# zeynelacikgoez/PyAudioLocalization

Hardware: AMD Instinct MI355X
Metric: mic-pair GCC-PHAT correlations/s @44.1kHz·1s (higher is better)
Workload: dtype f64; 1 GPU; metric run: 64 frame(s)/step/GPU x 64 mics x 44100 samples @ 44100 Hz, 2016 pairs/frame, max_expected_delay=0.05; n=88199 = 89 x 991: prime-factor inverse, Rader row DFTs (cyclic convolutions of 990 points in LDS) + dense column DFTs; mics=64, samples=44100, pairs_per_frame=2016, fused_column_statistics=default, finishing_column_pass=default, rader_columns=default, gather=none, split=frames, parallelism=frames sharded over 1 GPU(s)

## Files before the change

### pyaudiolocalization_amd/csrc/engine.h

```cpp
#pragma once
#include <hip/hip_runtime.h>

#include <cstdarg>
#include <cstdint>
#include <cstdio>
#include <map>
#include <string>
#include <tuple>
#include <vector>

#include "../../include/pal_hip.h"
#include "fin_scratch.h"
#include "fft_core.h"
#include "pair_route.h"
#include "plan_geometry.h"
#include "peak_types.h"
#include "resample_math.h"

namespace pal {

struct FinArgs;

struct Conv {
  ConvGeom g;
// ... 23 lines not shown
  int n = 0;
  int H = 0;
  int lin = 0;
  int nout = 0;
  cd* w = nullptr;
  Conv fwd;
  Conv inv;
  Pfa pfa;
  long long used = 0;
  size_t spec_stride() const { return pfa.on() ? size_t(pfa.rows()) * size_t(pfa.n2) : size_t(H); }
};

struct ProfileSlot {
  double ms = 0;
  int64_t launches = 0;
};

enum Ws : int {
  kWsWork = 0,
  kWsCorr = 1,
  kWsSpectra = 2,
  kWsQuads = 3,
  kWsStageIn = 4, kWsStageTable = 5, kWsStageOut = 6, kWsStagePairs = 15,
  kWsStatus = 7,
  kWsPeaks0 = 8, kWsPeaks1 = 9, kWsPeaks2 = 12,
  kWsBootRows = 10, kWsBootRound = 11, kWsBootPeaks = 13,
  kWsZeroRows = 14,
  kWsFin0 = 16, kWsFin1 = 17, kWsFin2 = 18,
  kWsFlags = 19, kWsFlagQuads = 20, kWsFlagTable = 21,
  kWsSolve = 22,
  kWsBlockTable = 23,
  kWsResample = 24,
  kWsClosure = 25,
  kWsCount = 26
};
constexpr Ws peak_scratch_slot(int slot) { return slot == 0 ? kWsPeaks0 : (slot == 1 ? kWsPeaks1 : kWsPeaks2); }
constexpr Ws fin_scratch_slot(int slot) { return Ws(kWsFin0 + slot); }

struct Engine {
  int device = 0;
  int cu_count = 256;
  hipStream_t stream = nullptr;
  hipStream_t stream2 = nullptr;
  hipStream_t stream3 = nullptr;
  hipStream_t stream_of(int slot) const { return slot == 0 ? stream : (slot == 1 ? stream2 : stream3); }
  hipEvent_t ev_fork = nullptr, ev_join2 = nullptr, ev_join3 = nullptr;
  hipEvent_t ev_fin = nullptr;
  int fin_serialize(hipStream_t on);
  int fin_done(hipStream_t on);
  bool fin_pending = false;
  bool fin_serial = false;
  bool rows_lean = true;
  long long rows_lean_min = 200000;
  bool lean_store = true;
  int debug_memo = 0;
  bool one_stream = false;
  PlanSwitches plan_sw;
  bool xcd_rows = true;
  bool rows_shared = true;
  std::string err;
  static constexpr int kDefaultChunk = 128;
  int chunk = kDefaultChunk;
  bool chunk_auto = true;
  int pair_group(int n) const {
    if (!chunk_auto) return chunk;
    const long long g = (1ll << 30) / (16ll * (n > 0 ? n : 1));
    return int(g < 32 ? 32 : (g > 240 ? 240 : g));
  }
  std::map<std::tuple<int, int, int>, Plan> plans;
  struct XConv { Conv conv; long long used = 0; };
// ... 70 lines not shown
  int solve_positions_impl(const pal_pair_record* d_tables, int B, int M, const int32_t* lengths, const double* mics, const double* calib,
                           const double* weights, const double* extra_starts, const pal_solve_params* prm, pal_position_record* out,
                           int loss, double f_scale, double* pair_weights);
  int tdoa_closure_dev(const pal_pair_record* d_tables, int B, int M, const int32_t* lengths, int32_t tol, int32_t min_votes, int32_t weight_mode,
                       int32_t* d_votes, int32_t* d_mic_closed, double* d_weights, pal_closure_frame* d_summary);
  int closure_check(int B, int M, const int32_t* lengths, int32_t tol, int32_t min_votes, int32_t weight_mode);
  int32_t* solve_idx = nullptr;
  int solve_idx_M = 0;
  std::vector<double> rs_win;
  std::vector<ResampleTap> rs_host;
  int rs_num_table = 0;
  double rs_ratio = 0;
  int peaks(const double* corr, size_t stride, int rows, int n, int n2, const pal_phat_params& prm,
            pal_pair_record* table, int32_t* ksel_multi, int slot);
  int peaks_setup(const double* corr, size_t stride, int rows, int n, int n2, const pal_phat_params& prm, int blocks, int grid_n2, int slot, PeakArgs& a);
  int peaks_finish(PeakArgs& a, int rows, pal_pair_record* table, int32_t* ksel_multi, int slot);
  int pfa_rows(const Plan& pl, const cd* permuted, const int4* quads, int G, cd* Y, hipStream_t on);
  int fin_setup(const Plan& pl, int rows, int nblk, int grid_rows, const pal_phat_params& prm, int n2, pal_pair_record* table,
                int* need, int slot, PeakArgs& a, struct FinArgs& fa, unsigned& nwg, int G);
  int rows_lean_group(const Plan& pl, const double* corr, size_t stride, int G, int rows, const pal_phat_params& prm, int n2,
                      pal_pair_record* table, int* need, int slot);
  int pfa_pair_group_fin(const Plan& pl, const cd* permuted, const int4* quads, int G, int rows, cd* Y, const int* zero_rows,
                         const pal_phat_params& prm, int n2, pal_pair_record* table, int* need, int slot,
                         double* corr = nullptr, size_t stride = 0);
  int pfa_pair_group_fused(const Plan& pl, const cd* permuted, const int4* quads, int G, int rows, cd* Y, double* corr, size_t stride,
                           const int* zero_rows, const pal_phat_params& prm, int n2, pal_pair_record* table, int32_t* ksel_multi, int slot);
  bool pfa_forward_applies(const Plan& pl, int len) const;
  int pfa_forward_spectra(Plan& pl, const double* frames, size_t frame_stride, int rows, int len, cd* spectra, const int* flags);
  bool pfa_forward = true;
  bool fin_cols = true;
  unsigned fin_epoch[3] = {};
  FinKey fin_key[3];
  unsigned fin_wrap = kFinEpochWrap;
  int fin_giveup = 0;
  bool fuse_peaks = true;
};

struct ProfScope {
  Engine* e;
  int slot;
  hipEvent_t a = nullptr;
  hipStream_t on;
  ProfScope(Engine* eng, const char* name, hipStream_t s = nullptr) : e(eng), slot(-1), on(s ? s : eng->stream) {
    if (e->profiling && e->prof_gate) {
      slot = e->prof_slot(name);
      e->prof_begin(slot, &a, on);
    }
  }
  ~ProfScope() {
    if (slot >= 0) e->prof_end(slot, a, on);
  }
};

#define PAL_TRY(expr)                \
  do {                               \
    int _rc = (expr);                \
    if (_rc != PAL_OK) return _rc;   \
  } while (0)

#define PAL_HIP(expr) PAL_TRY(check((expr), #expr))

}
```

### pyaudiolocalization_amd/csrc/pair_route.h

```cpp
#pragma once

namespace pal {

constexpr int kColsOwn = 62;

struct RouteIn {
  int n, nout; bool split; int n1, n2, nch, lm; bool r89;
  bool table, corr, multi; long long npairs;
  bool stored_only;
  int num_peaks, threshold_method; double threshold_multiplier;
  bool fin_cols, fuse_peaks, lean_store, rows_lean; long long rows_lean_min;
};

enum class RouteTransform { kFinish, kLeanStore, kFused, kPfa, kFourStep };
enum class RouteStats { kNone, kPass, kRowsLean, kThreeLaunches };

struct PairRoute {
  RouteTransform transform;
  RouteStats stats;
  bool flags_pairs() const { return transform == RouteTransform::kFinish || transform == RouteTransform::kLeanStore || stats == RouteStats::kRowsLean; }
};

inline int fin_blocks(int n2, int nch) { return (n2 + (nch <= 1 ? 4 : 1) * kColsOwn - 1) / ((nch <= 1 ? 4 : 1) * kColsOwn); }

inline bool nohist(int threshold_method, double threshold_multiplier) {
  return threshold_method > 0 || (threshold_multiplier >= 0 && threshold_multiplier <= 2.0);
}

inline PairRoute pair_route(const RouteIn& f) {
  const bool lean_peak = f.fin_cols && !f.stored_only && f.num_peaks == 1 && !f.multi;
  const bool no_hist = nohist(f.threshold_method, f.threshold_multiplier);
  const int nblk = fin_blocks(f.n2, f.nch);
  if (f.table && f.fuse_peaks && f.split && f.nch >= 1 && f.nch <= 4 && f.n2 >= 3) {
    bool cols_ok = f.r89 || (f.nch >= 2 && f.nch <= 4) || (f.nch <= 1 && f.lm <= 13);
    if (!f.r89 && nblk < 12) cols_ok = false;
    if (lean_peak && !f.corr && f.n2 >= 256 && cols_ok) return {RouteTransform::kFinish, RouteStats::kPass};
    if (f.lean_store && lean_peak && nblk >= 12 && no_hist) return {RouteTransform::kLeanStore, RouteStats::kPass};
    return {RouteTransform::kFused, RouteStats::kPass};
  }
  const RouteTransform tr = f.split ? RouteTransform::kPfa : RouteTransform::kFourStep;
  if (!f.table) return {tr, RouteStats::kNone};
  const bool lean = f.rows_lean && lean_peak && f.npairs >= f.rows_lean_min && no_hist && f.nout == f.n && f.n >= 4096 && f.n <= 50000;
  return {tr, lean ? RouteStats::kRowsLean : RouteStats::kThreeLaunches};
}

}
```

### pyaudiolocalization_amd/csrc/pal_api.hip

```cpp
#include <dlfcn.h>

#include <cmath>
#include <cstring>

#include "engine.h"

namespace pal {

static std::string g_create_error;

int Engine::fail(int code, const char* fmt, ...) {
  char buf[512];
  va_list ap;
  va_start(ap, fmt);
  vsnprintf(buf, sizeof buf, fmt, ap);
  va_end(ap);
  err = buf;
  return code;
}

int Engine::check(hipError_t e, const char* what) {
  if (e == hipSuccess) return PAL_OK;
  const int code = e == hipErrorOutOfMemory ? PAL_ERR_NOMEM : PAL_ERR_HIP;
  return fail(code, "%s: %s", what, hipGetErrorString(e));
// ... 264 lines not shown
  if (env) e->plan_sw.allow_pfa = atoi(env) != 0;
  env = getenv("PAL_RADER");
  if (env) e->plan_sw.allow_rader = atoi(env) != 0;
  env = getenv("PAL_PFA_BIG");
  if (env) e->plan_sw.allow_big = atoi(env) != 0;
  env = getenv("PAL_FOUR_REG");
  if (env) e->plan_sw.four_reg = atoi(env) != 0;
  env = getenv("PAL_XCD_ROWS");
  if (env) e->xcd_rows = atoi(env) != 0;
  env = getenv("PAL_ROWS_SHARED");
  if (env) e->rows_shared = atoi(env) != 0;
  env = getenv("PAL_PFA_FWD");
  if (env) e->pfa_forward = atoi(env) != 0;
  env = getenv("PAL_FUSED");
  if (env) e->fuse_peaks = atoi(env) != 0;
  env = getenv("PAL_R89");
  if (env) e->plan_sw.allow_r89 = atoi(env) != 0;
  env = getenv("PAL_FIN_SERIAL");
  if (env) e->fin_serial = atoi(env) != 0;
  env = getenv("PAL_FIN");
  if (env) e->fin_cols = atoi(env) != 0;
  env = getenv("PAL_ROWS_LEAN");
  if (env) e->rows_lean = atoi(env) != 0;
  env = getenv("PAL_PAIR_BLOCK");
  if (env) e->pair_block = atoi(env);
  env = getenv("PAL_ROWS_LEAN_MIN");
  if (env && atoll(env) >= 1) e->rows_lean_min = atoll(env);
  env = getenv("PAL_LEAN_STORE");
  if (env) e->lean_store = atoi(env) != 0;
  env = getenv("PAL_DEBUG_MEMO");
  if (env) e->debug_memo = atoi(env);
  env = getenv("PAL_DEBUG_FIN_WRAP");
  if (env && atoi(env) >= 2) e->fin_wrap = unsigned(atoi(env));
  env = getenv("PAL_DEBUG_FIN_GIVEUP");
  if (env) e->fin_giveup = atoi(env) != 0 ? 1 : 0;
  env = getenv("PAL_MAX_PLANS");
  if (env && atoi(env) >= 2) e->max_plans = atoi(env);
  *out = reinterpret_cast<pal_handle>(e);
  return PAL_OK;
}

void pal_destroy(pal_handle h) {
  if (!h) return;
  Engine* e = reinterpret_cast<Engine*>(h);
  hipSetDevice(e->device);
  pal_comm_destroy(h);
  (void)e->clear_plans();
  for (cd* p : e->stage_tw) if (p) hipFree(p);
  for (cd* p : e->stage_twc) if (p) hipFree(p);
  for (void* p : e->ws) if (p) hipFree(p);
  if (e->quads) hipFree(e->quads);
  if (e->quads_blk) hipFree(e->quads_blk);
  if (e->perm_blk) hipFree(e->perm_blk);
  if (e->solve_idx) hipFree(e->solve_idx);
  for (hipEvent_t ev : e->ev_pool) hipEventDestroy(ev);
  hipStreamDestroy(e->stream2);
  hipStreamDestroy(e->stream3);
  hipEventDestroy(e->ev_fork);
  hipEventDestroy(e->ev_join2);
  hipEventDestroy(e->ev_join3);
  hipEventDestroy(e->ev_fin);
  hipStreamDestroy(e->stream);
  delete e;
}

const char* pal_last_error(pal_handle h) {
// ... 468 lines not shown
```

### pyaudiolocalization_amd/csrc/pfa.hip

```cpp
#include <cmath>
#include <cstdlib>
#include <vector>

#include "pfa_kernels.h"
#include "pfa_rader.h"
#include "pfa_cols_stats.h"
#include "pfa_cols_fin.h"
#include "pfa_forward.h"
#include "pfa_big.h"

namespace pal {

#ifndef PAL_BIG13_PTS
#define PAL_BIG13_PTS 32
#endif
#ifndef PAL_BIG14_PTS
#define PAL_BIG14_PTS 32
#endif
constexpr int kBig13 = PAL_BIG13_PTS, kBig14 = PAL_BIG14_PTS;

static_assert(kColChunk == kPfaTC && kColUnroll == kPfaUnr && kRader89 == kR89, "plan_geometry.h against the column pass's constants");
static_assert(sizeof(RowStep) == sizeof(int2) && sizeof(Cplx) == sizeof(cd), "plan_geometry.h tables are uploaded as they are");

void Engine::free_pfa(Pfa& f) {
// ... 182 lines not shown
  return PAL_OK;
}

int Engine::fin_setup(const Plan& pl, int rows, int nblk, int grid_rows, const pal_phat_params& prm, int n2, pal_pair_record* table,
                      int* need, int slot, PeakArgs& a, FinArgs& fa, unsigned& nwg, int G) {
  const int n = pl.n;
  PAL_TRY(peaks_setup(nullptr, 0, rows, n, n2, prm, nblk, 0, slot, a));
  const FinLayout lay = fin_layout(pair_group(n), nblk, grid_rows);
  char* base = nullptr;
  PAL_TRY(scratch(fin_scratch_slot(slot), lay.total, &base));
  PAL_TRY(status_words(&fa.status));
  fa.table = table;
  fa.need = need;
  fa.done = reinterpret_cast<unsigned*>(base);
  FinKey key;
  key.gmax = pair_group(n);
  key.nblk = nblk;
  key.grid_rows = grid_rows;
  key.block = ws_bytes[fin_scratch_slot(slot)];
  if (fin_must_zero(fin_key[slot], key, fin_epoch[slot], fin_wrap)) {
    PAL_HIP(hipMemsetAsync(base, 0, key.block, stream_of(slot)));
    fin_key[slot] = key;
    fin_epoch[slot] = 0;
  }
  fa.epoch = ++fin_epoch[slot];
  fa.emax = reinterpret_cast<double*>(base + lay.off_emax);
  fa.parts = reinterpret_cast<FinPartial*>(base + lay.off_parts);
  fa.edge = reinterpret_cast<double*>(base + lay.off_edge);
  fa.giveup = fin_giveup;
  fa.pw = 1;
  fa.corr = nullptr;
  fa.stride = 0;
  fa.store_rows = 0;
  fa.windowed = std::isnan(prm.max_expected_delay) ? 0 : 1;
  fa.win_lo = 1;
  fa.win_hi = n - 2;
  if (fa.windowed) {
    const double med = prm.max_expected_delay, fs = prm.fs;
    long long k = -1;
    if (med >= 0) {
      const double est = med * fs;
      k = est < double(n) ? (long long)est + 2 : (long long)n;
      while (k >= 0 && !(std::fabs(double(k) / fs) <= med)) --k;
    }
    if (k < 0) { fa.win_lo = 1; fa.win_hi = 0; }
    else {
      const long long lo = (long long)(n2 - 1) - k, hi = (long long)(n2 - 1) + k;
      fa.win_lo = int(lo < 1 ? 1 : lo);
      fa.win_hi = int(hi > n - 2 ? n - 2 : hi);
    }
  }
  fa.cheb = a.method == 0 && nohist(prm.threshold_method, prm.threshold_multiplier) ? 1 : 0;
  nwg = 8u * unsigned((G + 7) / 8) * unsigned(nblk);
  return PAL_OK;
}

int Engine::rows_lean_group(const Plan& pl, const double* corr, size_t stride, int G, int rows, const pal_phat_params& prm, int n2,
                            pal_pair_record* table, int* need, int slot) {
  constexpr int NS = 22;
  const hipStream_t on = stream_of(slot);
  const int chunks = (pl.n + kColsOwn - 1) / kColsOwn;
  const int nblk = (chunks + 4 * NS - 1) / (4 * NS);
  PeakArgs a;
  FinArgs fa;
  unsigned nwg = 0;
  PAL_TRY(fin_setup(pl, rows, nblk, 1, prm, n2, table, need, slot, a, fa, nwg, G));
  fa.pw = 4;
  fa.corr = const_cast<double*>(corr);
  fa.stride = stride;
  ProfScope ps(this, "k_rows_lean", on);
  k_rows_lean<NS><<<dim3(nwg), dim3(256), 0, on>>>(corr, stride, G, nblk, a, fa, rows);
  PAL_HIP(hipGetLastError());
  return PAL_OK;
}

int Engine::pfa_pair_group_fin(const Plan& pl, const cd* permuted, const int4* quads, int G, int rows, cd* Y, const int* zero_rows,
                               const pal_phat_params& prm, int n2, pal_pair_record* table, int* need, int slot,
                               double* corr, size_t stride) {
  const Pfa& f = pl.pfa;
  const hipStream_t on = stream_of(slot);
  const bool shortcols = f.nch <= 1;
  const int nblk = fin_blocks(f.n2, f.nch);
  PeakArgs a;
  FinArgs fa;
  unsigned nwg = 0;
  PAL_TRY(fin_setup(pl, rows, nblk, f.n1, prm, n2, table, need, slot, a, fa, nwg, G));
  fa.corr = corr;
  fa.stride = stride;
  fa.store_rows = corr ? 1 : 0;
  PAL_TRY(pfa_rows(pl, permuted, quads, G, Y, on));
  {
    ProfScope ps(this, corr ? "k_pfa_cols_lean" : "k_pfa_cols_fin", on);
    const dim3 grid(nwg);
    const bool full = (f.n1 - 1) / 2 == f.nch * kPfaTC;
    const bool hist = !(a.method > 0 || fa.cheb);
    const int nw = f.nch == 2 ? 2 : (f.nch == 3 && !hist ? 3 : 4);
    FinSrc src{Y, f.T, static_cast<const Rader89Tab*>(f.r89_tab)};
    PAL_TRY(fin_serialize(on));
#define PAL_COLS_FIN(MODE, HI, FU, NW) k_pfa_cols_fin<MODE, kPfaTC, kPfaUnr, HI, FU, NW><<<grid, dim3(64 * NW), 0, on>>>(src, f.n1, f.n2, G, f.nch, nblk, zero_rows, a, fa, rows)
#define PAL_COLS_FIN_FU(MODE, HI, NW) do { if (full) PAL_COLS_FIN(MODE, HI, true, NW); else PAL_COLS_FIN(MODE, HI, false, NW); } while (0)
    if (!hist) fa.pw = shortcols ? 4 : nw;
    if (shortcols) { if (hist) PAL_COLS_FIN(kColsStrips, true, false, 4); else PAL_COLS_FIN(kColsStrips, false, false, 4); }
    else if (f.r89 && full && nw == 4) { if (hist) PAL_COLS_FIN(kColsRader89, true, true, 4); else PAL_COLS_FIN(kColsRader89, false, true, 4); }
    else if (nw == 3) PAL_COLS_FIN_FU(kColsDense, false, 3);
    else if (nw == 2) { if (hist) PAL_COLS_FIN_FU(kColsDense, true, 2); else PAL_COLS_FIN_FU(kColsDense, false, 2); }
    else { if (hist) PAL_COLS_FIN_FU(kColsDense, true, 4); else PAL_COLS_FIN_FU(kColsDense, false, 4); }
#undef PAL_COLS_FIN_FU
#undef PAL_COLS_FIN
    PAL_HIP(hipGetLastError());
    PAL_TRY(fin_done(on));
  }
  return PAL_OK;
}

}
```

### pyaudiolocalization_amd/csrc/pfa_cols_fin.h

```cpp
#pragma once
#include <climits>

#include "fin_scratch.h"
#include "pfa_cols_stats.h"
#include "reduce.h"
#include "wave_reduce.h"

namespace pal {

struct FinPartial {
  double vmin, hb, plat;
  double s1, s2, a1;
  double hw, platw;
  double hm;
  double w1, w2;
  int mb, mw, mm, pad;
};
static_assert(sizeof(FinPartial) == 104 && sizeof(FinPartial) == kFinPartialBytes, "thirteen words (fin_scratch.h)");

struct FinArgs {
  pal_pair_record* table;
  int* need;
  unsigned* done;
  double* edge;
  double* emax;
  unsigned epoch;
  int giveup;
  FinPartial* parts;
  int* status;
  int win_lo, win_hi;
  int windowed;
  int pw;
  double* corr;
  size_t stride;
  int store_rows;
  int cheb;
};

struct FinWave {
  double vmax, hb, hw, hm, plat, platw, nvmin, s1, s2, a1, w1, w2;
  int imax, mb, mw, mm;
};

struct FinShared {
  unsigned hwin[2 * kWin];
  int swin0[144];
  FinWave wave[4];
};
static_assert(sizeof(FinShared) <= 2 * (kLogBins + 1) * sizeof(unsigned), "the finish scratch aliases the histograms");
static_assert(alignof(FinShared) <= 16, "(the histograms' storage is 16-byte aligned)");

__device__ __forceinline__ unsigned ld_agent(const unsigned* p) { return __hip_atomic_load(p, __ATOMIC_RELAXED, __HIP_MEMORY_SCOPE_AGENT); }
__device__ __forceinline__ int ld_agent(const int* p) { return __hip_atomic_load(p, __ATOMIC_RELAXED, __HIP_MEMORY_SCOPE_AGENT); }
__device__ __forceinline__ double ld_agent(const double* p) {
  return __longlong_as_double(__hip_atomic_load(reinterpret_cast<const long long*>(p), __ATOMIC_RELAXED, __HIP_MEMORY_SCOPE_AGENT));
}
__device__ __forceinline__ void st_agent(unsigned* p, unsigned v) { __hip_atomic_store(p, v, __ATOMIC_RELAXED, __HIP_MEMORY_SCOPE_AGENT); }
__device__ __forceinline__ void st_agent(double* p, double v) {
  __hip_atomic_store(reinterpret_cast<long long*>(p), __double_as_longlong(v), __ATOMIC_RELAXED, __HIP_MEMORY_SCOPE_AGENT);
}
template <class T> __device__ __forceinline__ void st_words(T* dst, const T& v) {
  static_assert(sizeof(T) % 8 == 0, "whole words");
  const long long* src = reinterpret_cast<const long long*>(&v);
  long long* d = reinterpret_cast<long long*>(dst);
#pragma unroll
  for (int k = 0; k < int(sizeof(T) / 8); ++k) __hip_atomic_store(d + k, src[k], __ATOMIC_RELAXED, __HIP_MEMORY_SCOPE_AGENT);
}
template <class T> __device__ __forceinline__ T ld_words(const T* src) {
  T v;
// ... 250 lines not shown
        e += v;
      }
      have = f1 >= 0 && f2 >= 0;
      if (have) {
        b1lo = log_bin_floor(w0 + f1); b1hi = log_bin_floor(w0 + f1 + 1);
        b2lo = log_bin_floor(w0 + f2); b2hi = log_bin_floor(w0 + f2 + 1);
      }
    }
    __syncthreads();
    if (have) {
      const double ml_ = r2 != r1 ? (b1lo + b2lo) * 0.5 : b1lo, mh_ = r2 != r1 ? (b1hi + b2hi) * 0.5 : b1hi;
      tlo = pa.mult >= 0 ? pa.mult * ml_ : pa.mult * mh_;
      thi = pa.mult >= 0 ? pa.mult * mh_ : pa.mult * ml_;
    } else {
      flag = true;
      why |= 16;
    }
  }
  fin_decide(pa, fa, row, s, flag, why, interval, tlo, thi, tid == 0);
}

}
#include "pfa_fin_lean.h"
namespace pal {

enum { kColsDense = 0, kColsRader89 = 1, kColsStrips = 2 };

struct FinSrc {
  const cd* Y;
  const double* T;
  const Rader89Tab* tab;
};

template <int MODE, int TC, int UNR, bool HIST, bool FULL, int NW>
__global__ __launch_bounds__(64 * NW) __attribute__((amdgpu_waves_per_eu(MODE == kColsRader89 ? 3 : 2))) void k_pfa_cols_fin(FinSrc src, int N1, int N2, int G, int nch, int nblk,
                                                      const int* __restrict__ zero_rows, PeakArgs pa, FinArgs fa, int rows) {
  constexpr bool R89 = MODE == kColsRader89, STRIPS = MODE == kColsStrips;
  static_assert(!R89 || (NW == 4 && FULL), "the Rader column transform is the four-wavefront N1 = 89 case");
  static_assert(!HIST || NW <= 4, "the histogram form merges at most four wavefronts per block");
  const cd* __restrict__ Y = src.Y;
  const double* __restrict__ T = src.T;
  const Rader89Tab* __restrict__ tab = src.tab;
  constexpr int kHistDoubles = (2 * (kLogBins + 1) * int(sizeof(unsigned)) + 7) / 8;
  __shared__ __attribute__((aligned(16))) double lds_big[R89 ? 88 * 64 : kHistDoubles];
  unsigned (*const hist)[kLogBins + 1] = reinterpret_cast<unsigned (*)[kLogBins + 1]>(lds_big);
  __shared__ FinPartial res[4][2];
  __shared__ double wmax[4][2];
  __shared__ unsigned wtot[4][2];
  __shared__ int medbin[2];
  __shared__ int s_imax[2];
  __shared__ int s_flag;
  const int tid = threadIdx.x, lane = tid & 63;
  const int wave = __builtin_amdgcn_readfirstlane(tid >> 6);
  const int ch = STRIPS ? 0 : wave;
  const int xs = int(blockIdx.x & 7u), slot = int(blockIdx.x >> 3);
  const int cb = slot % nblk, g = xs + 8 * (slot / nblk);
  if (g >= G) return;
  const int strips = STRIPS ? nblk * NW : nblk, strip = STRIPS ? cb * NW + wave : cb;
  const int nact = STRIPS ? NW : nch;
  const int c_lo = int((long long)strip * N2 / strips), c_hi = int((long long)(strip + 1) * N2 / strips);
  const bool active = STRIPS ? true : ch < nch;
  const int m2 = c_lo - 1 + lane;
  const bool live = m2 >= 0 && m2 < N2 && lane <= c_hi - c_lo + 1;
  const bool own = live && lane >= 1 && lane <= c_hi - c_lo;
  const bool inner = own && m2 >= 1 && m2 <= N2 - 2;
  const int m2c = m2 < 0 ? 0 : (m2 < N2 ? m2 : N2 - 1);
  const int h = (N1 - 1) / 2;
  const int n = pa.n;
  constexpr bool want_median = HIST;
  constexpr int LANES = 64 * NW;
  if (want_median && !R89) {
    unsigned* hz = &hist[0][0];
// ... 1 lines not shown
  }
  constexpr int TCD = R89 ? 1 : TC;
  double cx[TCD], sy[TCD], cy[TCD], sx[TCD];
  double sumx = 0, sumy = 0;
  cd y0 = mk(0, 0);
  cd ro[R89 ? kR89Slots : 1];
  cd c0 = mk(0, 0);
  const double kp = zero_rows && zero_rows[2 * g] ? 0.0 : 1.0, kq = zero_rows && 2 * g + 1 < rows && zero_rows[2 * g + 1] ? 0.0 : 1.0;
  int slot_t = 0;
  if constexpr (R89) {
    slot_t = tab->tmap[wave][lane < kR89Slots ? lane : 0];
    r89_columns(Y + size_t(g) * N1 * N2 + m2c, N2, wave, lane, tab, lds_big, ro, c0);
    if (want_median) {
      unsigned* hz = &hist[0][0];
      for (int q = tid; q < 2 * (kLogBins + 1); q += LANES) hz[q] = 0;
    }
    if (kp == 0.0 || kq == 0.0) {
      c0.x *= kp; c0.y *= kq;
#pragma unroll
      for (int i = 0; i < kR89Slots; ++i) { ro[i].x *= kp; ro[i].y *= kq; }
    }
  } else {
    if (active) pfa_cols_accumulate<TC, UNR>(Y + size_t(g) * N1 * N2 + m2c, N1, N2, nch, ch, T, y0, cx, sy, cy, sx, sumx, sumy);
    if (kp == 0.0) { y0.x = sumx = 0.0; }
    if (kq == 0.0) { y0.y = sumy = 0.0; }
#pragma unroll
    for (int tt = 0; tt < TCD; ++tt) {
      cx[tt] *= kp; sy[tt] *= kp; cy[tt] *= kq; sx[tt] *= kq;
    }
  }
  if constexpr (!HIST) {
    bool last;
    if constexpr (R89) {
      last = fin_lean_r89<true, false, kR89Slots>(ro, c0, slot_t, 0u, wave, lane, g, cb, nblk, N1, N2, rows, c_lo, m2, own, inner, cb == 0 || cb == nblk - 1,
                                                  -1, true, pa, fa);
    } else {
      static_assert(R89 || 2 * TCD == kR89Slots, "22 slots per wavefront");
      cd zs[kR89Slots];
      const cd z0 = mk(y0.x + sumx, y0.y + sumy);
      unsigned emask = active && ch == 0 ? 1u : 0u;
#pragma unroll
      for (int tt = 0; tt < TCD; ++tt) {
        zs[tt] = mk(y0.x + cx[tt] - sy[tt], y0.y + cy[tt] + sx[tt]);
        zs[TCD + tt] = mk(y0.x + cx[tt] + sy[tt], y0.y + cy[tt] - sx[tt]);
        if (active && (FULL || ch * TC + tt + 1 <= h)) emask |= (1u << (1 + tt)) | (1u << (1 + TCD + tt));
      }
      const int tl = ch * TC + (lane < TCD ? lane : lane - TCD) + 1;
      const int st = lane < TCD ? tl : N1 - tl;
      last = fin_lean_r89<false, false, kR89Slots>(zs, z0, st, emask, wave, lane, g, cb, nblk, N1, N2, rows, c_lo, m2, own, inner,
                                                   active && (c_lo == 0 || c_hi == N2), -1, true, pa, fa);
    }
    if (!last) return;
    if (wave != 0) return;
    fin_rows_wave(pa, fa, g, nblk, rows, N1, N2, lane);
    return;
  }
  auto each_sample = [&](int r, auto&& fn) {
    if constexpr (R89) {
      fn([&]() { return r ? c0.y : c0.x; }, 0, wave == 0);
#pragma unroll
      for (int i = 0; i < kR89Slots; ++i) fn([&]() { return r ? ro[i].y : ro[i].x; }, __builtin_amdgcn_readlane(slot_t, i), true);
    } else {
      const double base = r ? y0.y : y0.x;
      fn([&]() { return base + (r ? sumy : sumx); }, 0, ch == 0);
#pragma unroll
      for (int tt = 0; tt < TCD; ++tt) {
        const int t = ch * TC + tt + 1;
        fn([&]() { return r ? base + cy[tt] + sx[tt] : base + cx[tt] - sy[tt]; }, t, FULL || t <= h);
      }
#pragma unroll
      for (int tt = TCD - 1; tt >= 0; --tt) {
        const int t = ch * TC + tt + 1;
        fn([&]() { return r ? base + cy[tt] - sx[tt] : base + cx[tt] + sy[tt]; }, N1 - t, FULL || t <= h);
      }
    }
  };
  __syncthreads();

  const int nrow = 2 * g + 1 < rows ? 2 : 1;
  constexpr unsigned kBase4 = unsigned(1023 * 128 - kLogBins) * 4u, kTop4 = kBase4 + unsigned(kLogBins - 1) * 4u;
  const unsigned lift = own ? 0u : unsigned(kLogBins) * 4u;
  const unsigned one = 1u;
#pragma unroll
  for (int r = 0; r < 2; ++r) {
    double vm = -INFINITY, vn = INFINITY, s1 = 0, s2 = 0, a1 = 0;
    int tm = 0;
    if (active && r < nrow) {
// ... 317 lines not shown
```

### pyaudiolocalization_amd/csrc/pfa_fin_lean.h

```cpp
#pragma once

namespace pal {

__device__ __forceinline__ double wave_max63r(double v) { return wave_reduce_d(v, -__builtin_huge_val(), [](double a, double b) { return max_raw(a, b); }); }
__device__ __forceinline__ double wave_min63r(double v) { return wave_reduce_d(v, __builtin_huge_val(), [](double a, double b) { return min_raw(a, b); }); }
__device__ __forceinline__ double readlane_d(double v, int l) {
  return __hiloint2double(__builtin_amdgcn_readlane(__double2hiint(v), l), __builtin_amdgcn_readlane(__double2loint(v), l));
}

template <class BETTER> __device__ __forceinline__ void uniform_arg_sparse(double& v, int& i, BETTER better) {
  const unsigned long long cm = __ballot(i >= 0);
  if (cm == 0) { i = -1; v = 0; return; }
  if ((cm & (cm - 1)) == 0) {
    const int l = int(__builtin_ctzll(cm));
    v = readlane_d(v, l);
    i = __builtin_amdgcn_readlane(i, l);
    return;
  }
  wave_arg63(v, i, better);
  v = wave_bcast63(v);
  i = wave_bcast63(i);
}
__device__ __forceinline__ void uniform_arg_dense_hi(double& v, int& i) {
  const double h = wave_bcast63(wave_max63r(i >= 0 ? v : -__builtin_huge_val()));
// ... 22 lines not shown
  v = h;
}
__device__ __forceinline__ double uniform_max_sparse(double v) {
  if (__ballot(v > -__builtin_huge_val()) == 0) return -__builtin_huge_val();
  return wave_bcast63(wave_max63r(v));
}

constexpr int kQuadXor1 = 0xB1, kQuadXor2 = 0x4E, kRor4 = 0x124, kRor8 = 0x128;
template <class OP> __device__ __forceinline__ double wave_pair_reduce(double a, double b, OP op) {
  const bool odd = threadIdx.x & 1;
  double c = odd ? b : a;
  const double d = odd ? a : b;
  c = op(c, dpp_d<kQuadXor1>(0.0, d));
  c = op(c, dpp_d<kQuadXor2>(0.0, c));
  c = op(c, dpp_d<kRor4>(0.0, c));
  c = op(c, dpp_d<kRor8>(0.0, c));
  {
    const unsigned lo = unsigned(__double2loint(c)), hi = unsigned(__double2hiint(c));
    const auto l = __builtin_amdgcn_permlane16_swap(lo, lo, false, false);
    const auto h = __builtin_amdgcn_permlane16_swap(hi, hi, false, false);
    c = op(__hiloint2double(int(h[0]), int(l[0])), __hiloint2double(int(h[1]), int(l[1])));
  }
  {
    const unsigned lo = unsigned(__double2loint(c)), hi = unsigned(__double2hiint(c));
    const auto l = __builtin_amdgcn_permlane32_swap(lo, lo, false, false);
    const auto h = __builtin_amdgcn_permlane32_swap(hi, hi, false, false);
    c = op(__hiloint2double(int(h[0]), int(l[0])), __hiloint2double(int(h[1]), int(l[1])));
  }
  return c;
}
__device__ __forceinline__ double wave_pair_sum(double a, double b) { return wave_pair_reduce(a, b, [](double x, double y) { return x + y; }); }
__device__ __forceinline__ double wave_pair_min(double a, double b) { return wave_pair_reduce(a, b, [](double x, double y) { return min_raw(x, y); }); }

template <bool ALL, bool PART, int NS>
__device__ __forceinline__ bool fin_lean_r89(const cd (&ro)[NS], const cd c0, const int slot_t, const unsigned emask, const int wave, const int lane,
                                             const int g, const int cb, const int nblk, const int N1, const int N2, const int rows, const int c_lo,
                                             const int m2, const bool own, const bool inner, const bool edge_block, const int pslot, const bool pvalid,
                                             const PeakArgs& pa, const FinArgs& fa) {
  static_assert(NS + 1 <= 32, "slot masks are 32 bits");
  const int n = pa.n, S = pa.splits, PW = fa.pw;
  const unsigned long long pvm = PART ? __ballot(pvalid) : ~0ull;
  const unsigned long long ownm = __ballot(own), innerm = __ballot(inner);
  const int nrow = 2 * g + 1 < rows ? 2 : 1;
  const bool windowed = fa.windowed != 0;
  auto T = [&](int slot) { return slot == 0 ? 0 : __builtin_amdgcn_readlane(slot_t, slot - 1); };
  auto for_slots = [&](int r, auto&& fn) {
    if (ALL ? wave == 0 : (emask & 1u) != 0) fn(r ? c0.y : c0.x, 0);
#pragma unroll
    for (int i = 0; i < NS; ++i)
      if (ALL || (emask >> (i + 1) & 1u)) fn(r ? ro[i].y : ro[i].x, i + 1);
  };
  auto slot_mask = [&](int t_lo, int t_hi) -> unsigned {
    const unsigned long long b = __ballot(lane < NS && slot_t >= t_lo && slot_t <= t_hi);
    const unsigned m = (unsigned(b) << 1) | (t_lo <= 0 && t_hi >= 0 ? 1u : 0u);
    return ALL ? (wave == 0 ? m : m & ~1u) : m & emask;
  };
  int lo1 = 1, hi1 = 0;
  unsigned wmask = 0;
  if (windowed) {
    const int elo = fa.win_lo - (pa.dist - 1), ehi = fa.win_hi + (pa.dist - 1);
    lo1 = elo > 1 ? elo : 1;
    hi1 = ehi < n - 2 ? ehi : n - 2;
    if (lo1 <= hi1) wmask = slot_mask(lo1 / N2, hi1 / N2);
  }

  double vn[2], s1[2], s2[2], a1[2];
  FinPartial pt[2];
#pragma unroll
  for (int r = 0; r < 2; ++r) {
    vn[r] = INFINITY; s1[r] = s2[r] = a1[r] = 0;
    pt[r].hb = 0; pt[r].plat = -INFINITY; pt[r].hw = 0; pt[r].platw = -INFINITY; pt[r].hm = 0;
    pt[r].mb = pt[r].mw = pt[r].mm = -1; pt[r].pad = 0;
// ... 76 lines not shown
      pt[r].hw = hq; pt[r].mw = mq; pt[r].hm = hg; pt[r].mm = mg;
      pt[r].platw = uniform_max_sparse(platw);
    }
  }

  if (edge_block) {
    const bool mine = own && (m2 <= 1 || m2 >= N2 - 2);
    if (__ballot(mine)) {
      const int e = m2 <= 1 ? m2 : 3 - (N2 - 1 - m2);
#pragma unroll
      for (int r = 0; r < 2; ++r) {
        if (r >= nrow) continue;
        double* dst = fa.edge + (size_t(2 * g + r) * 4 + (mine ? e : 0)) * N1;
        for_slots(r, [&](double x, int slot) {
          if (mine) st_agent(dst + T(slot), x);
        });
      }
    }
  }

  const bool stored = fa.corr != nullptr;
  if (stored && fa.store_rows) {
#pragma unroll
    for (int r = 0; r < 2; ++r) {
      if (r >= nrow) continue;
      double* const out = fa.corr + size_t(2 * g + r) * fa.stride + m2;
      for_slots(r, [&](double x, int slot) {
        const int t = T(slot);
        if (own && (!PART || N2 * t + m2 < n)) out[size_t(N2) * t] = x;
      });
    }
  }

  const double rmin = wave_pair_min(vn[0], vn[1]);
  const double r1 = wave_pair_sum(s1[0], s1[1]), r2 = wave_pair_sum(s2[0], s2[1]), ra = wave_pair_sum(a1[0], a1[1]);

  double w1[2] = {0, 0}, w2[2] = {0, 0};
  bool gave_up = false;
  bool have_w[2] = {false, false};
#pragma unroll
  for (int r = 0; r < 2; ++r) {
    if (r >= nrow || stored) continue;
    const int row = 2 * g + r;
    double bv = -INFINITY;
    int bi = -1;
    const double* em = fa.emax + size_t(row) * S * PW * 2;
    const double want = double(fa.epoch);
    bool late = fa.giveup != 0;
    for (int q = lane; !fa.giveup && q < S * PW; q += 64) {
      double v = 0, code = 0;
      int spins = 0;
      for (;;) {
        ld_agent16(em + 2 * q, v, code);
        if (floor(code / kEpochUnit) == want) break;
        if (++spins > kSpinLimit) { late = true; break; }
        __builtin_amdgcn_s_sleep(8);
      }
      const int i = int(code - want * kEpochUnit) - 1;
      if (!late && i >= 0 && i < n && (bi < 0 || arg_better<0>(v, i, bv, bi))) { bv = v; bi = i; }
    }
    if (__ballot(late)) { gave_up = true; continue; }
    uniform_arg_dense_lo(bv, bi);
    int imax = bi;
    if (imax < 0 || imax >= n) imax = 0;
    const int A = imax - pa.snr_w > 0 ? imax - pa.snr_w : 0, B = imax + pa.snr_w < n ? imax + pa.snr_w : n;
    const int tA = A / N2, tB = (B - 1) / N2;
    const unsigned smask = slot_mask(tA, tB);
    if (smask == 0) continue;
    have_w[r] = true;
    const bool inA = m2 >= A - tA * N2, inB = m2 < B - tB * N2;
    double u1 = 0, u2 = 0;
    for_slots(r, [&](double x, int slot) {
      if (!(smask >> slot & 1u)) return;
      const int t = T(slot);
      const bool in = own && (t > tA || inA) && (t < tB || inB);
      const double xm = in ? x : 0.0;
      u1 += xm;
      u2 = __builtin_fma(xm, xm, u2);
    });
    w1[r] = u1; w2[r] = u2;
  }
  if (gave_up && lane == 0) atomicAdd(fa.status + kStGaveUp, 1);

  {
    double q1 = 0, q2 = 0;
    if (have_w[0] || have_w[1]) { q1 = wave_pair_sum(w1[0], w1[1]); q2 = wave_pair_sum(w2[0], w2[1]); }
    if (lane < nrow) {
      FinPartial o;
      const bool second = lane == 1;
      o.hb = second ? pt[1].hb : pt[0].hb; o.plat = second ? pt[1].plat : pt[0].plat;
      o.hw = second ? pt[1].hw : pt[0].hw; o.platw = second ? pt[1].platw : pt[0].platw; o.hm = second ? pt[1].hm : pt[0].hm;
      o.mb = second ? pt[1].mb : pt[0].mb; o.mw = second ? pt[1].mw : pt[0].mw; o.mm = second ? pt[1].mm : pt[0].mm;
      o.vmin = rmin; o.s1 = r1; o.s2 = r2; o.a1 = ra; o.w1 = q1; o.w2 = q2;
      o.pad = gave_up ? 1 : 0;
      st_words(fa.parts + (size_t(2 * g + lane) * S + cb) * PW + wave, o);
    }
  }
  stores_done();
  if (lane == 0) st_agent(fa.done + (size_t(g) * nblk + cb) * PW + wave, fa.epoch);
  return cb == nblk - 1;
}


__device__ __forceinline__ void fin_row_wave(const PeakArgs& pa, const FinArgs& fa, int row, int N1, int N2, int lane) {
  const int S = pa.splits, n = pa.n, P = S * fa.pw;
  const bool windowed = fa.windowed != 0;
  FinRow s;
  {
    const double* em = fa.emax + size_t(row) * P * 2;
    for (int q = lane; q < P; q += 64) {
      const double v = ld_agent(em + 2 * q);
      const int i = int(ld_agent(em + 2 * q + 1) - double(fa.epoch) * kEpochUnit) - 1;
      if (i >= 0 && i < n && (s.imax < 0 || arg_better<0>(v, i, s.vmax, s.imax))) { s.vmax = v; s.imax = i; }
    }
  }
  for (int q = lane; q < P; q += 64) {
    const FinPartial pt = ld_words(fa.parts + size_t(row) * P + q);
    s.vmin = fmin(s.vmin, pt.vmin);
    if (pt.mb >= 0 && (s.mb < 0 || higher(pt.hb, pt.mb, s.hb, s.mb))) { s.hb = pt.hb; s.mb = pt.mb; }
    s.plat = fmax(s.plat, pt.plat);
    s.s1 += pt.s1; s.s2 += pt.s2; s.a1 += pt.a1;
    s.w1 += pt.w1; s.w2 += pt.w2;
    s.abandoned = s.abandoned || pt.pad != 0;
    if (windowed) {
      if (pt.mw >= 0 && (s.mw < 0 || higher(pt.hw, pt.mw, s.hw, s.mw))) { s.hw = pt.hw; s.mw = pt.mw; }
      if (pt.mm >= 0 && (s.mm < 0 || higher(pt.hm, pt.mm, s.hm, s.mm))) { s.hm = pt.hm; s.mm = pt.mm; }
      s.platw = fmax(s.platw, pt.platw);
    }
  }
  const double* E = fa.edge + size_t(row) * 4 * N1;
  for (int k = lane; k < 2 * N1; k += 64) {
    const bool first = k < N1;
    const int t = first ? k : k - N1;
    const int m = first ? N2 * t : N2 * t + N2 - 1;
    if (m < 1 || m > n - 2) continue;
    const double x = ld_agent(first ? E + t : E + 3 * N1 + t);
// ... 7 lines not shown
    if (tie && (inw || inm)) s.platw = fmax(s.platw, x);
    if (pk && (s.mb < 0 || higher(x, m, s.hb, s.mb))) { s.hb = x; s.mb = m; }
    if (pk && inw && (s.mw < 0 || higher(x, m, s.hw, s.mw))) { s.hw = x; s.mw = m; }
    if (pk && inm && (s.mm < 0 || higher(x, m, s.hm, s.mm))) { s.hm = x; s.mm = m; }
  }
  uniform_arg_dense_lo(s.vmax, s.imax);
  uniform_arg_dense_hi(s.hb, s.mb);
  if (windowed) {
    uniform_arg_dense_hi(s.hw, s.mw);
    uniform_arg_sparse(s.hm, s.mm, [](double v1, int i1, double v2, int i2) { return higher(v1, i1, v2, i2); });
    s.platw = uniform_max_sparse(s.platw);
  }
  s.plat = uniform_max_sparse(s.plat);
  s.vmin = wave_bcast63(wave_min63r(s.vmin));
  s.s1 = wave_bcast63(wave_sum63(s.s1)); s.s2 = wave_bcast63(wave_sum63(s.s2)); s.a1 = wave_bcast63(wave_sum63(s.a1));
  s.w1 = wave_bcast63(wave_sum63(s.w1)); s.w2 = wave_bcast63(wave_sum63(s.w2));

  bool flag = false;
  int why = 0;
  if (s.imax < 0 || s.imax >= n) { s.imax = 0; flag = true; why |= 1; }
  if (__ballot(s.abandoned) != 0) { flag = true; why |= 1; }
  if (fa.corr) {
    const int lo = s.imax - pa.snr_w > 0 ? s.imax - pa.snr_w : 0, hi = s.imax + pa.snr_w < n ? s.imax + pa.snr_w : n;
    const double* rowp = fa.corr + size_t(row) * fa.stride;
    double u1 = 0, u2 = 0;
    for (int k = lo + lane; k < hi; k += 64) {
      const double x = ld_agent(rowp + k);
      u1 += x;
      u2 = __builtin_fma(x, x, u2);
    }
    s.w1 = wave_bcast63(wave_sum63(u1));
    s.w2 = wave_bcast63(wave_sum63(u2));
  }
  fin_decide(pa, fa, row, s, flag, why, false, 0, 0, lane == 0);
}

__device__ __forceinline__ void fin_rows_wave(const PeakArgs& pa, const FinArgs& fa, int g, int nblk, int rows, int N1, int N2, int lane) {
  bool late = fa.giveup != 0;
  for (int q = lane; !fa.giveup && q < nblk * fa.pw; q += 64) {
    int spins = 0;
    while (ld_agent(fa.done + size_t(g) * nblk * fa.pw + q) != fa.epoch) {
      if (++spins > kSpinLimit) { late = true; break; }
      __builtin_amdgcn_s_sleep(8);
    }
  }
  if (__ballot(late)) {
    if (lane < 2 && 2 * g + lane < rows) { fa.need[2 * g + lane] = 1; atomicAdd(fa.status + kStFlagged, 1); atomicAdd(fa.status + kStGaveUp, 1); }
    return;
  }
#pragma nounroll
  for (int r = 0; r < 2; ++r)
    if (2 * g + r < rows) fin_row_wave(pa, fa, 2 * g + r, N1, N2, lane);
}

}
```

Measured before the change: 1.671 million pair-correlations/s.

## Store correlation strips near the delay window and compute SNR windows from them

In the lean finishing column pass, each wavefront now writes the correlation samples that can fall inside the SNR window of a windowed peak (three pieces around the lag window edges) into a per-slot strip buffer. The per-row finisher then computes the SNR window sums from that strip. If the window is not covered by the strip, it recomputes the samples directly from the column grid with an N1-point DFT. This replaces the speculative per-wavefront window statistics (the w1/w2 accumulation and its reduction around candidate peaks), trading them for extra global stores to a scratch buffer and a possible slow direct fallback. The new path is on by default and can be turned off with PAL_FIN_STRIP.

```diff
diff --git a/pyaudiolocalization_amd/csrc/engine.h b/pyaudiolocalization_amd/csrc/engine.h
--- a/pyaudiolocalization_amd/csrc/engine.h
+++ b/pyaudiolocalization_amd/csrc/engine.h
@@ -79,10 +79,12 @@
   kWsBlockTable = 23,
   kWsResample = 24,
   kWsClosure = 25,
-  kWsCount = 26
+  kWsFinStrip0 = 26, kWsFinStrip1 = 27, kWsFinStrip2 = 28,
+  kWsCount = 29
 };
 constexpr Ws peak_scratch_slot(int slot) { return slot == 0 ? kWsPeaks0 : (slot == 1 ? kWsPeaks1 : kWsPeaks2); }
 constexpr Ws fin_scratch_slot(int slot) { return Ws(kWsFin0 + slot); }
+constexpr Ws fin_strip_slot(int slot) { return Ws(kWsFinStrip0 + slot); }
 
 struct Engine {
   int device = 0;
@@ -219,6 +221,7 @@
   unsigned fin_epoch[3] = {};
   FinKey fin_key[3];
   unsigned fin_wrap = kFinEpochWrap;
+  bool fin_strip_on = true;
   int fin_giveup = 0;
   bool fuse_peaks = true;
 };
diff --git a/pyaudiolocalization_amd/csrc/pair_route.h b/pyaudiolocalization_amd/csrc/pair_route.h
--- a/pyaudiolocalization_amd/csrc/pair_route.h
+++ b/pyaudiolocalization_amd/csrc/pair_route.h
@@ -44,4 +44,70 @@
   return {tr, lean ? RouteStats::kRowsLean : RouteStats::kThreeLaunches};
 }
 
+
+#if defined(__HIPCC__) || defined(__CUDACC__)
+#define PAL_ROUTE_HD __host__ __device__
+#else
+#define PAL_ROUTE_HD
+#endif
+
+constexpr double kFinStripShare = 0.34;
+constexpr int kFinStripPieces = 3;
+
+struct FinStrip {
+  int pieces;
+  int lo[kFinStripPieces], hi[kFinStripPieces];
+  int base[kFinStripPieces];
+  int len;
+  bool on() const { return pieces > 0; }
+};
+
+inline FinStrip fin_no_strip() {
+  FinStrip s;
+  s.pieces = 0;
+  s.len = 0;
+  for (int p = 0; p < kFinStripPieces; ++p) { s.lo[p] = 1; s.hi[p] = 0; s.base[p] = 0; }
+  return s;
 }
+
+inline FinStrip fin_strip(int n, bool windowed, int win_lo, int win_hi, int snr_w, bool lean_finish, bool enabled) {
+  FinStrip s = fin_no_strip();
+  if (!enabled || !lean_finish || !windowed || win_lo > win_hi || n < 1 || snr_w < 1) return s;
+  const long long D = ((long long)win_hi - win_lo + 1) / 2;
+  long long lo[3] = {0, (long long)win_lo - snr_w, (long long)n - D - snr_w};
+  long long hi[3] = {D + snr_w - 1, (long long)win_hi + snr_w - 1, (long long)n - 1};
+  long long total = 0;
+  for (int p = 0; p < 3; ++p) {
+    if (lo[p] < 0) lo[p] = 0;
+    if (hi[p] > n - 1) hi[p] = n - 1;
+    if (s.pieces > 0 && lo[p] <= (long long)s.hi[s.pieces - 1] + 1) {
+      if (hi[p] > s.hi[s.pieces - 1]) { total += hi[p] - s.hi[s.pieces - 1]; s.hi[s.pieces - 1] = int(hi[p]); }
+      continue;
+    }
+    s.lo[s.pieces] = int(lo[p]);
+    s.hi[s.pieces] = int(hi[p]);
+    s.base[s.pieces] = int(total);
+    total += hi[p] - lo[p] + 1;
+    ++s.pieces;
+  }
+  if (double(total) > kFinStripShare * double(n)) return fin_no_strip();
+  s.len = int(total);
+  return s;
+}
+
+PAL_ROUTE_HD inline int fin_strip_offset(const FinStrip& s, int m) {
+  int off = -1;
+  for (int p = 0; p < kFinStripPieces; ++p) off = m >= s.lo[p] && m <= s.hi[p] ? s.base[p] + (m - s.lo[p]) : off;
+  return off;
+}
+PAL_ROUTE_HD inline int fin_strip_window(const FinStrip& s, int lo, int hi) {
+  int off = -1;
+  for (int p = 0; p < kFinStripPieces; ++p) off = lo < hi && lo >= s.lo[p] && hi - 1 <= s.hi[p] ? s.base[p] + (lo - s.lo[p]) : off;
+  return off;
+}
+PAL_ROUTE_HD inline void fin_snr_window(int imax, int snr_w, int n, int& lo, int& hi) {
+  lo = imax - snr_w > 0 ? imax - snr_w : 0;
+  hi = imax + snr_w < n ? imax + snr_w : n;
+}
+
+}
diff --git a/pyaudiolocalization_amd/csrc/pal_api.hip b/pyaudiolocalization_amd/csrc/pal_api.hip
--- a/pyaudiolocalization_amd/csrc/pal_api.hip
+++ b/pyaudiolocalization_amd/csrc/pal_api.hip
@@ -320,6 +320,8 @@
   if (env) e->debug_memo = atoi(env);
   env = getenv("PAL_DEBUG_FIN_WRAP");
   if (env && atoi(env) >= 2) e->fin_wrap = unsigned(atoi(env));
+  env = getenv("PAL_FIN_STRIP");
+  if (env) e->fin_strip_on = atoi(env) != 0;
   env = getenv("PAL_DEBUG_FIN_GIVEUP");
   if (env) e->fin_giveup = atoi(env) != 0 ? 1 : 0;
   env = getenv("PAL_MAX_PLANS");
diff --git a/pyaudiolocalization_amd/csrc/pfa.hip b/pyaudiolocalization_amd/csrc/pfa.hip
--- a/pyaudiolocalization_amd/csrc/pfa.hip
+++ b/pyaudiolocalization_amd/csrc/pfa.hip
@@ -238,6 +238,11 @@
   fa.corr = nullptr;
   fa.stride = 0;
   fa.store_rows = 0;
+  fa.strip = nullptr;
+  fa.st = fin_no_strip();
+  fa.grid = nullptr;
+  fa.roots = nullptr;
+  fa.zero_rows = nullptr;
   fa.windowed = std::isnan(prm.max_expected_delay) ? 0 : 1;
   fa.win_lo = 1;
   fa.win_hi = n - 2;
@@ -302,8 +307,19 @@
     const bool hist = !(a.method > 0 || fa.cheb);
     const int nw = f.nch == 2 ? 2 : (f.nch == 3 && !hist ? 3 : 4);
     FinSrc src{Y, f.T, static_cast<const Rader89Tab*>(f.r89_tab)};
+    const FinStrip st = fin_strip(pl.n, fa.windowed != 0, fa.win_lo, fa.win_hi, a.snr_w, !corr && !hist, fin_strip_on);
+    if (st.on()) {
+      PAL_TRY(scratch(fin_strip_slot(slot), size_t(2 * pair_group(pl.n)) * size_t(st.len) * sizeof(double), &fa.strip));
+      fa.st = st;
+      fa.grid = Y;
+      fa.roots = f.r1;
+      fa.zero_rows = zero_rows;
+    }
+    const bool strip = fa.strip != nullptr;
     PAL_TRY(fin_serialize(on));
-#define PAL_COLS_FIN(MODE, HI, FU, NW) k_pfa_cols_fin<MODE, kPfaTC, kPfaUnr, HI, FU, NW><<<grid, dim3(64 * NW), 0, on>>>(src, f.n1, f.n2, G, f.nch, nblk, zero_rows, a, fa, rows)
+#define PAL_COLS_FIN(MODE, HI, FU, NW) do { \
+      if (!HI && strip) k_pfa_cols_fin<MODE, kPfaTC, kPfaUnr, HI, FU, NW, !HI><<<grid, dim3(64 * NW), 0, on>>>(src, f.n1, f.n2, G, f.nch, nblk, zero_rows, a, fa, rows); \
+      else k_pfa_cols_fin<MODE, kPfaTC, kPfaUnr, HI, FU, NW, false><<<grid, dim3(64 * NW), 0, on>>>(src, f.n1, f.n2, G, f.nch, nblk, zero_rows, a, fa, rows); } while (0)
 #define PAL_COLS_FIN_FU(MODE, HI, NW) do { if (full) PAL_COLS_FIN(MODE, HI, true, NW); else PAL_COLS_FIN(MODE, HI, false, NW); } while (0)
     if (!hist) fa.pw = shortcols ? 4 : nw;
     if (shortcols) { if (hist) PAL_COLS_FIN(kColsStrips, true, false, 4); else PAL_COLS_FIN(kColsStrips, false, false, 4); }
diff --git a/pyaudiolocalization_amd/csrc/pfa_cols_fin.h b/pyaudiolocalization_amd/csrc/pfa_cols_fin.h
--- a/pyaudiolocalization_amd/csrc/pfa_cols_fin.h
+++ b/pyaudiolocalization_amd/csrc/pfa_cols_fin.h
@@ -2,6 +2,7 @@
 #include <climits>
 
 #include "fin_scratch.h"
+#include "pair_route.h"
 #include "pfa_cols_stats.h"
 #include "reduce.h"
 #include "wave_reduce.h"
@@ -35,6 +36,11 @@
   size_t stride;
   int store_rows;
   int cheb;
+  double* strip;
+  FinStrip st;
+  const cd* grid;
+  const cd* roots;
+  const int* zero_rows;
 };
 
 struct FinWave {
@@ -351,12 +357,13 @@
   const Rader89Tab* tab;
 };
 
-template <int MODE, int TC, int UNR, bool HIST, bool FULL, int NW>
+template <int MODE, int TC, int UNR, bool HIST, bool FULL, int NW, bool STRIP = false>
 __global__ __launch_bounds__(64 * NW) __attribute__((amdgpu_waves_per_eu(MODE == kColsRader89 ? 3 : 2))) void k_pfa_cols_fin(FinSrc src, int N1, int N2, int G, int nch, int nblk,
                                                       const int* __restrict__ zero_rows, PeakArgs pa, FinArgs fa, int rows) {
   constexpr bool R89 = MODE == kColsRader89, STRIPS = MODE == kColsStrips;
   static_assert(!R89 || (NW == 4 && FULL), "the Rader column transform is the four-wavefront N1 = 89 case");
   static_assert(!HIST || NW <= 4, "the histogram form merges at most four wavefronts per block");
+  static_assert(!(HIST && STRIP), "the strip form belongs to the per-wavefront statistics");
   const cd* __restrict__ Y = src.Y;
   const double* __restrict__ T = src.T;
   const Rader89Tab* __restrict__ tab = src.tab;
@@ -424,7 +431,7 @@
   if constexpr (!HIST) {
     bool last;
     if constexpr (R89) {
-      last = fin_lean_r89<true, false, kR89Slots>(ro, c0, slot_t, 0u, wave, lane, g, cb, nblk, N1, N2, rows, c_lo, m2, own, inner, cb == 0 || cb == nblk - 1,
+      last = fin_lean_r89<true, false, kR89Slots, STRIP>(ro, c0, slot_t, 0u, wave, lane, g, cb, nblk, N1, N2, rows, c_lo, m2, own, inner, cb == 0 || cb == nblk - 1,
                                                   -1, true, pa, fa);
     } else {
       static_assert(R89 || 2 * TCD == kR89Slots, "22 slots per wavefront");
@@ -439,12 +446,12 @@
       }
       const int tl = ch * TC + (lane < TCD ? lane : lane - TCD) + 1;
       const int st = lane < TCD ? tl : N1 - tl;
-      last = fin_lean_r89<false, false, kR89Slots>(zs, z0, st, emask, wave, lane, g, cb, nblk, N1, N2, rows, c_lo, m2, own, inner,
+      last = fin_lean_r89<false, false, kR89Slots, STRIP>(zs, z0, st, emask, wave, lane, g, cb, nblk, N1, N2, rows, c_lo, m2, own, inner,
                                                    active && (c_lo == 0 || c_hi == N2), -1, true, pa, fa);
     }
     if (!last) return;
     if (wave != 0) return;
-    fin_rows_wave(pa, fa, g, nblk, rows, N1, N2, lane);
+    fin_rows_wave<STRIP>(pa, fa, g, nblk, rows, N1, N2, lane);
     return;
   }
   auto each_sample = [&](int r, auto&& fn) {
diff --git a/pyaudiolocalization_amd/csrc/pfa_fin_lean.h b/pyaudiolocalization_amd/csrc/pfa_fin_lean.h
--- a/pyaudiolocalization_amd/csrc/pfa_fin_lean.h
+++ b/pyaudiolocalization_amd/csrc/pfa_fin_lean.h
@@ -78,12 +78,13 @@
 __device__ __forceinline__ double wave_pair_sum(double a, double b) { return wave_pair_reduce(a, b, [](double x, double y) { return x + y; }); }
 __device__ __forceinline__ double wave_pair_min(double a, double b) { return wave_pair_reduce(a, b, [](double x, double y) { return min_raw(x, y); }); }
 
-template <bool ALL, bool PART, int NS>
+template <bool ALL, bool PART, int NS, bool STRIP = false>
 __device__ __forceinline__ bool fin_lean_r89(const cd (&ro)[NS], const cd c0, const int slot_t, const unsigned emask, const int wave, const int lane,
                                              const int g, const int cb, const int nblk, const int N1, const int N2, const int rows, const int c_lo,
                                              const int m2, const bool own, const bool inner, const bool edge_block, const int pslot, const bool pvalid,
                                              const PeakArgs& pa, const FinArgs& fa) {
   static_assert(NS + 1 <= 32, "slot masks are 32 bits");
+  static_assert(!(STRIP && PART), "row chunks read stored rows: their finisher reads the SNR window from the row");
   const int n = pa.n, S = pa.splits, PW = fa.pw;
   const unsigned long long pvm = PART ? __ballot(pvalid) : ~0ull;
   const unsigned long long ownm = __ballot(own), innerm = __ballot(inner);
@@ -226,6 +227,25 @@
     }
   }
 
+  if constexpr (STRIP) {
+    unsigned smask = 0;
+#pragma unroll
+    for (int p = 0; p < kFinStripPieces; ++p)
+      if (p < fa.st.pieces) smask |= slot_mask(fa.st.lo[p] / N2, fa.st.hi[p] / N2);
+    if (smask) {
+#pragma unroll
+      for (int r = 0; r < 2; ++r) {
+        if (r >= nrow) continue;
+        double* const dst = fa.strip + size_t(2 * g + r) * fa.st.len;
+        for_slots(r, [&](double x, int slot) {
+          if (!(smask >> slot & 1u)) return;
+          const int off = fin_strip_offset(fa.st, m2 + N2 * T(slot));
+          if (own && off >= 0) st_agent(dst + off, x);
+        });
+      }
+    }
+  }
+
   const double rmin = wave_pair_min(vn[0], vn[1]);
   const double r1 = wave_pair_sum(s1[0], s1[1]), r2 = wave_pair_sum(s2[0], s2[1]), ra = wave_pair_sum(a1[0], a1[1]);
 
@@ -234,7 +254,7 @@
   bool have_w[2] = {false, false};
 #pragma unroll
   for (int r = 0; r < 2; ++r) {
-    if (r >= nrow || stored) continue;
+    if (STRIP || r >= nrow || stored) continue;
     const int row = 2 * g + r;
     double bv = -INFINITY;
     int bi = -1;
@@ -278,7 +298,7 @@
 
   {
     double q1 = 0, q2 = 0;
-    if (have_w[0] || have_w[1]) { q1 = wave_pair_sum(w1[0], w1[1]); q2 = wave_pair_sum(w2[0], w2[1]); }
+    if (!STRIP && (have_w[0] || have_w[1])) { q1 = wave_pair_sum(w1[0], w1[1]); q2 = wave_pair_sum(w2[0], w2[1]); }
     if (lane < nrow) {
       FinPartial o;
       const bool second = lane == 1;
@@ -296,6 +316,30 @@
 }
 
 
+__device__ __forceinline__ void fin_window_direct(const FinArgs& fa, int row, int N1, int N2, int lo, int hi, int lane, double& u1, double& u2) {
+  const cd* const Yg = fa.grid + size_t(row >> 1) * N1 * N2;
+  const bool imag = row & 1;
+  const double keep = fa.zero_rows && fa.zero_rows[row] ? 0.0 : 1.0;
+#pragma nounroll
+  for (int k = lo + lane; k < hi; k += 64) {
+    const int t = k / N2;
+    const cd* col = Yg + (k - t * N2);
+    double acc = 0;
+    int q = 0;
+#pragma unroll 8
+    for (int j = 0; j < N1; ++j) {
+      const cd y = col[size_t(j) * N2], w = fa.roots[q];
+      acc = imag ? __builtin_fma(y.y, w.x, __builtin_fma(-y.x, w.y, acc)) : __builtin_fma(y.x, w.x, __builtin_fma(y.y, w.y, acc));
+      q += t;
+      q = q >= N1 ? q - N1 : q;
+    }
+    const double x = acc * keep;
+    u1 += x;
+    u2 = __builtin_fma(x, x, u2);
+  }
+}
+
+template <bool STRIP>
 __device__ __forceinline__ void fin_row_wave(const PeakArgs& pa, const FinArgs& fa, int row, int N1, int N2, int lane) {
   const int S = pa.splits, n = pa.n, P = S * fa.pw;
   const bool windowed = fa.windowed != 0;
@@ -369,9 +413,28 @@
     s.w1 = wave_bcast63(wave_sum63(u1));
     s.w2 = wave_bcast63(wave_sum63(u2));
   }
+  if constexpr (STRIP) {
+    int lo, hi;
+    fin_snr_window(s.imax, pa.snr_w, n, lo, hi);
+    double u1 = 0, u2 = 0;
+    const int off = fin_strip_window(fa.st, lo, hi);
+    if (off >= 0) {
+      const double* sp = fa.strip + size_t(row) * fa.st.len + off;
+      for (int k = lane; k < hi - lo; k += 64) {
+        const double x = ld_agent(sp + k);
+        u1 += x;
+        u2 = __builtin_fma(x, x, u2);
+      }
+    } else {
+      fin_window_direct(fa, row, N1, N2, lo, hi, lane, u1, u2);
+    }
+    s.w1 = wave_bcast63(wave_sum63(u1));
+    s.w2 = wave_bcast63(wave_sum63(u2));
+  }
   fin_decide(pa, fa, row, s, flag, why, false, 0, 0, lane == 0);
 }
 
+template <bool STRIP = false>
 __device__ __forceinline__ void fin_rows_wave(const PeakArgs& pa, const FinArgs& fa, int g, int nblk, int rows, int N1, int N2, int lane) {
   bool late = fa.giveup != 0;
   for (int q = lane; !fa.giveup && q < nblk * fa.pw; q += 64) {
@@ -387,7 +450,7 @@
   }
 #pragma nounroll
   for (int r = 0; r < 2; ++r)
-    if (2 * g + r < rows) fin_row_wave(pa, fa, 2 * g + r, N1, N2, lane);
-}
-
-}
+    if (2 * g + r < rows) fin_row_wave<STRIP>(pa, fa, 2 * g + r, N1, N2, lane);
+}
+
+}
```

After: 1.756 million pair-correlations/s (median of 6 runs). 1.05x the previous value.
